# PytorchConnectomics/pytorch_connectomics

Measured on AMD Instinct MI355X. Metric: voxels/s (train + sliding-window infer), MedNeXt-S 112^3 bf16, higher is better.
Workload: dtype bf16; 1 GPU; Lucchi++ sliding-window inference (configs[1]): MedNeXt-S k3, 165x1024x768 volume, roi 112^3, overlap 0.5, bump blending, sw_batch_size 8, random-init weights; step = one whole-volume EagerSlidingWindowEngine call (TTA off); value = window-voxels/s; sw_batch_size=8, window_pipeline_streams=3

## Files before the change

### include/pytc_hip.h

```cpp
#ifndef PYTC_HIP_H
#define PYTC_HIP_H

#include <stdint.h>

#ifdef __cplusplus
extern "C" {
#endif

#define PYTC_ABI_VERSION 5

#define PYTC_OK 0
#define PYTC_ERR_INVALID 1
#define PYTC_ERR_HIP 2
#define PYTC_ERR_UNSUPPORTED 3

#define PYTC_F32 0
#define PYTC_BF16 1

#define PYTC_VIEW_FLIP_Z 1
#define PYTC_VIEW_FLIP_Y 2
#define PYTC_VIEW_FLIP_X 4
#define PYTC_VIEW_SWAP_YX 8
#define PYTC_VIEW_SWAP_ZY 16
#define PYTC_VIEW_SWAP_ZX 32
// ... 80 lines not shown
#define PYTC_NORM_MINMAX 2
#define PYTC_NORM_DIVIDE 3
int64_t pytc_window_normalize_ws_elems(int B, int64_t n);
int pytc_window_normalize(float* x, int B, int64_t n, int mode, int binarize, float threshold, float divide, const float* clip,
                          double* workspace, void* stream);


int pytc_dwconv3d_stat_slots(int N, int D, int H, int W, int C, int K, int stride, int dtype,
                             int transposed);

int pytc_dwconv3d_kernel_variant(int N, int D, int H, int W, int C, int K, int stride, int dtype, int transposed);

int pytc_dwconv3d_fwd(const void* x, void* y, const float* w, const float* bias, float* stats,
                      int N, int D, int H, int W, int C, int K, int stride, int dtype,
                      void* stream);

int pytc_dwconv3d_fwd_wide(const void* x, void* y, const float* w, const float* bias, float* stats, int N, int D, int H,
                           int W, int C, int K, int stride, int dtype, void* stream);

int pytc_dwconv3d_res_supported(int D, int H, int W, int C, int K, int stride, int dtype);

int pytc_dwmix_supported(int D, int H, int W, int C, int C_hid, int C_out, int dtype);
int pytc_dwmix_fwd(const void* x, const float* taps, const float* dw_bias, const void* w2n, const float* b2n, const void* w3_f16,
                   const float* b3, int residual, void* y, const void* head_w, const float* head_b, float* head_y, int n_head, int N,
                   int D, int H, int W, int C, int C_hid, int C_out, int dtype, void* stream);
int pytc_dwconv3d_fwd_res(const void* x, const void* res, void* y, const float* w, const float* bias, int N, int D, int H,
                          int W, int C, int K, int stride, int dtype, void* stream);

int pytc_dwconvT3d_fwd(const void* x, void* y, const float* w, const float* bias, float* stats,
                       int N, int D, int H, int W, int C, int K, int dtype, void* stream);
// ... 325 lines not shown
```

### pytorch_connectomics_amd/_native.py

```python
from __future__ import annotations

import ctypes as C
import os
from pathlib import Path

LIB_PATH = Path(__file__).resolve().parent / "lib" / "libpytc_hip.so"
ABI_VERSION = 5

F32, BF16 = 0, 1
OK = 0

VIEW_FLIP_Z, VIEW_FLIP_Y, VIEW_FLIP_X, VIEW_SWAP_YX, VIEW_SWAP_ZY, VIEW_SWAP_ZX = 1, 2, 4, 8, 16, 32
VIEW_SWAPS = {VIEW_SWAP_YX: (1, 2), VIEW_SWAP_ZY: (0, 1), VIEW_SWAP_ZX: (0, 2)}
PAD_MODES = {"constant": 0, "reflect": 1, "replicate": 2, "circular": 3}
BLEND_PRODUCT, BLEND_MIN = 0, 1
ACT_NONE, ACT_SIGMOID, ACT_TANH, ACT_GELU, ACT_SOFTMAX, ACT_RELU, ACT_LEAKY, ACT_ELU = 0, 1, 2, 3, 4, 5, 6, 7
RES_NONE, RES_ADD, RES_UPSAMPLE, RES_GELU_BWD, RES_NORM_BWD = 0, 1, 2, 3, 4


class PwArgs(C.Structure):
    _fields_ = [
        ("x", C.c_void_p), ("w_packed", C.c_void_p), ("bias", C.c_void_p), ("ab", C.c_void_p),
        ("res", C.c_void_p), ("y", C.c_void_p),
        ("N", C.c_int), ("rows_per_sample", C.c_int64),
# ... 43 lines not shown
    "pytc_gather_windows": (C.c_int, [C.c_void_p, C.c_int, C.c_int, C.c_int, C.c_int, C.POINTER(C.c_int32),
                                      C.c_int, C.c_int, C.c_int, C.c_int, C.c_int, C.c_int, C.c_float,
                                      C.c_void_p, C.c_int, C.c_void_p]),
    "pytc_blend_accumulate": (C.c_int, [C.c_void_p, C.c_int, C.c_int, C.POINTER(C.c_int32), C.c_int, C.c_int,
                                        C.c_int, C.c_int, C.c_int, C.c_void_p, C.c_void_p, C.c_void_p, C.c_int,
                                        C.c_float, C.POINTER(C.c_int32), C.c_void_p, C.c_void_p, C.c_int, C.c_int,
                                        C.c_int, C.c_void_p]),
    "pytc_blend_finalize": (C.c_int, [C.c_void_p, C.c_void_p, C.c_int, C.c_int64, C.c_float, C.c_int, C.c_void_p]),
    "pytc_channel_activation": (C.c_int, [C.c_void_p, C.c_int, C.c_int64, C.c_int, C.c_int, C.c_int, C.c_int,
                                          C.c_float, C.c_void_p]),
    "pytc_ensemble_update": (C.c_int, [C.c_void_p, C.c_void_p, C.c_int64, C.c_int, C.c_int, C.c_void_p]),
    "pytc_dwconv3d_stat_slots": (C.c_int, [C.c_int] * 9),
    "pytc_dwconv3d_kernel_variant": (C.c_int, [C.c_int] * 9),
    "pytc_dwconv3d_fwd": (C.c_int, [C.c_void_p, C.c_void_p, C.c_void_p, C.c_void_p, C.c_void_p] + [C.c_int] * 8
                          + [C.c_void_p]),
    "pytc_dwconv3d_fwd_wide": (C.c_int, [C.c_void_p, C.c_void_p, C.c_void_p, C.c_void_p, C.c_void_p] + [C.c_int] * 8
                               + [C.c_void_p]),
    "pytc_dwconv3d_res_supported": (C.c_int, [C.c_int] * 7),
    "pytc_dwmix_supported": (C.c_int, [C.c_int] * 7),
    "pytc_dwmix_fwd": (C.c_int, [C.c_void_p] * 7 + [C.c_int] + [C.c_void_p] * 4 + [C.c_int] * 9 + [C.c_void_p]),
    "pytc_dwconv3d_fwd_res": (C.c_int, [C.c_void_p, C.c_void_p, C.c_void_p, C.c_void_p, C.c_void_p] + [C.c_int] * 8
                              + [C.c_void_p]),
    "pytc_dwconvT3d_fwd": (C.c_int, [C.c_void_p, C.c_void_p, C.c_void_p, C.c_void_p, C.c_void_p] + [C.c_int] * 7
                           + [C.c_void_p]),
    "pytc_groupnorm_finalize": (C.c_int, [C.c_void_p, C.c_int, C.c_float, C.c_void_p, C.c_void_p, C.c_float,
                                          C.c_void_p, C.c_int, C.c_int, C.c_void_p]),
    "pytc_groupnorm_fold_mlp": (C.c_int, [C.c_void_p, C.c_int, C.c_float, C.c_void_p, C.c_void_p, C.c_float, C.c_void_p,
                                          C.c_void_p, C.c_void_p, C.c_void_p, C.c_void_p, C.c_int, C.c_int, C.c_int, C.c_void_p]),
    "pytc_pw_gemm_supported": (C.c_int, [C.c_int, C.c_int]),
    "pytc_pw_gemm_fwd": (C.c_int, [C.c_void_p, C.c_void_p, C.c_void_p, C.c_void_p, C.c_void_p, C.c_int, C.c_int64, C.c_int, C.c_int,
# ... 248 lines not shown
```

### pytorch_connectomics_amd/csrc/dwconv_kernels.hip

```cpp
#include <type_traits>
#include "pytc_common.h"
#include "dwconv_march.h"

namespace pytc {

struct DwGeom {
  int N, D, H, W, C, K, stride, Do, Ho, Wo;
  int lpv;
  int vs;
  int iters;
  int slots;
  int cell;
  int xblock;
};

template <int VEC>
__device__ __forceinline__ void block_stats_reduce(float (&s1)[VEC], float (&s2)[VEC], int cv, int vslot,
                                                   bool active, const DwGeom& g, float* __restrict__ stats,
                                                   int n, int slot, float* lds) {
  const int C = g.C;
  if (active) {
#pragma unroll
    for (int i = 0; i < VEC; ++i) {
      lds[(vslot * 2 + 0) * C + cv * VEC + i] = s1[i];
// ... 1103 lines not shown
template <typename T>
static int dispatch_vec(int vec, bool transposed, const void* x, void* y, const float* w, const float* bias,
                        float* stats, const DwGeom& g, hipStream_t s) {
  switch (vec) {
    case 8: if constexpr (sizeof(T) == 2) return launch_dw<T, 8>(transposed, x, y, w, bias, stats, g, s); else break;
    case 4: return launch_dw<T, 4>(transposed, x, y, w, bias, stats, g, s);
    case 2: return launch_dw<T, 2>(transposed, x, y, w, bias, stats, g, s);
    case 1: return launch_dw<T, 1>(transposed, x, y, w, bias, stats, g, s);
  }
  set_error("dwconv3d: bad vector width %d", vec);
  return PYTC_ERR_INVALID;
}

static int dw_entry(bool transposed, const void* x, void* y, const float* w, const float* bias, float* stats,
                    int N, int D, int H, int W, int C, int K, int stride, int dtype, void* stream,
                    const void* res = nullptr, bool wide_range = false) {
  PYTC_REQUIRE(x && w, "dwconv3d: null pointer");
  if (res) {
    PYTC_REQUIRE(y && !stats, "dwconv3d_res: needs an output and takes no statistics");
    if (dtype != PYTC_BF16 || !march_ok(D, H, W, C, K, stride, dtype, transposed)) {
      set_error("dwconv3d_res: bf16 only, shape outside the z-march kernel (N=%d D=%d H=%d W=%d C=%d K=%d stride=%d)", N, D, H, W, C, K, stride);
      return PYTC_ERR_UNSUPPORTED;
    }
  }
  PYTC_REQUIRE(N >= 1 && D >= 1 && H >= 1 && W >= 1 && C >= 1, "dwconv3d: bad shape");
  PYTC_REQUIRE(stride == 1 || stride == 2, "dwconv3d: stride must be 1 or 2");
  PYTC_REQUIRE(dtype == PYTC_F32 || dtype == PYTC_BF16, "dwconv3d: bad dtype");
  PYTC_REQUIRE(!(wide_range && stats), "dwconv3d_fwd_wide: the gradient entry computes no statistics");
  DwTTile tt;
  const bool tt_form = transposed && K == 3 && dtype == PYTC_BF16 && (C == 64 || C == 128) && tuning_get("dwconvT_tile", 1) != 0 &&
                       dwconvT_tile_plan(tt, N, D, H, W, C);
// ... 15 lines not shown
    return PYTC_OK;
  }
  if (!transposed && K == 3 && stride == 2 && dtype == PYTC_BF16 && y && tuning_get("dwconv_s2_march", 1) != 0) {
    DwS2 t2;
    if (dwconv_s2_plan(t2, N, D, H, W, C)) {
      dwconv_s2_launch(x, y, w, bias, stats, t2, (hipStream_t)stream);
      PYTC_LAUNCH_CHECK("dwconv3d_k3_s2_march");
      return PYTC_OK;
    }
  }
  if (!res && !wide_range && mfma_small_ok(D, H, W, C, K, stride, dtype, transposed)) {
    DwMarch t;
    make_march(t, N, D, H, W, C, TILE_X);
    t.swizzle = tuning_get("dwconv_xcd_swizzle", 1);
    t.cg_inner = tuning_get("dwconv_cg_inner", 1);
    dwconv_mfma_launch(x, y, w, bias, stats, t, tuning_get("dwconv_mfma_variant", 0) | 1, (hipStream_t)stream);
    PYTC_LAUNCH_CHECK("dwconv3d_k3_mfma");
    return PYTC_OK;
  }
  if (march_ok(D, H, W, C, K, stride, dtype, transposed)) {
    DwMarch t;
    const bool wide_tile = !res && !wide_range && tuning_get("dwconv_march_h16", 1) != 0 && march_tile_x(W, dtype) == 16;
    make_march(t, N, D, H, W, C, wide_tile ? 16 : TILE_X);
    dim3 grid((unsigned)((long)t.slots * (C / MARCH_CG) * N)), block(wide_tile ? 512 : 256);
    t.swizzle = tuning_get("dwconv_xcd_swizzle", 1);
  t.cg_inner = tuning_get("dwconv_cg_inner", 1);
    if (dtype == PYTC_BF16 && !res && !wide_range && tuning_get("dwconv_mfma", 1) != 0) {
      dwconv_mfma_launch(x, y, w, bias, stats, t, tuning_get("dwconv_mfma_variant", 0), (hipStream_t)stream);
      PYTC_LAUNCH_CHECK("dwconv3d_k3_mfma");
      return PYTC_OK;
    }
    const int variant = tuning_get("dwconv_march_variant", 0);
#define PYTC_MARCH(PP, WW) \
  hipLaunchKernelGGL((dwconv3d_k3_march_kernel<bf16_t, 2, PP, true, WW>), grid, block, 0, (hipStream_t)stream, \
                     (const bf16_t*)x, (bf16_t*)y, w, bias, stats, t)
    const int h16 = (res || wide_range) ? 0 : tuning_get("dwconv_march_h16", 1);
    if (res) {
      if (h16)
        hipLaunchKernelGGL((dwconv3d_k3_march_kernel<bf16_t, 2, 3, true, 3, true, true>), grid, block, 0, (hipStream_t)stream,
                           (const bf16_t*)x, (bf16_t*)y, w, bias, stats, t, (const bf16_t*)res);
      else
        hipLaunchKernelGGL((dwconv3d_k3_march_kernel<bf16_t, 2, 3, true, 3, true>), grid, block, 0, (hipStream_t)stream,
                           (const bf16_t*)x, (bf16_t*)y, w, bias, stats, t, (const bf16_t*)res);
// ... 68 lines not shown
  DwGeom g;
  int vec;
  if (!make_geom(g, N, D, H, W, C, K, stride, dtype, transposed, vec)) return -1;
  if (transposed && K == 3 && dtype == PYTC_BF16 && (C == 64 || C == 128) && tuning_get("dwconvT_tile", 1) != 0) return 7;
  if (!transposed && K == 3 && stride == 2 && dtype == PYTC_BF16 && (C == 32 || C == 64) && tuning_get("dwconv_s2_march", 1) != 0) return 8;
  if (transposed) return g.cell ? 4 : 5;
  const size_t taps = (size_t)K * K * K * C * sizeof(float);
  if ((K == 3 || K == 5 || K == 7) && taps <= 64 * 1024 && tuning_get("dwconv_gather", 1) != 0)
    return (vec == 8 && stride == 1 && g.xblock) ? 2 : 1;
  return 0;
}

extern "C" int pytc_dwconv3d_fwd(const void* x, void* y, const float* w, const float* bias, float* stats, int N,
                                 int D, int H, int W, int C, int K, int stride, int dtype, void* stream) {
  return dw_entry(false, x, y, w, bias, stats, N, D, H, W, C, K, stride, dtype, stream);
}

extern "C" int pytc_dwconv3d_fwd_wide(const void* x, void* y, const float* w, const float* bias, float* stats, int N,
                                      int D, int H, int W, int C, int K, int stride, int dtype, void* stream) {
  return dw_entry(false, x, y, w, bias, stats, N, D, H, W, C, K, stride, dtype, stream, nullptr, true);
}

extern "C" int pytc_dwconv3d_res_supported(int D, int H, int W, int C, int K, int stride, int dtype) {
  return (dtype == PYTC_BF16 && march_ok(D, H, W, C, K, stride, dtype, 0)) ? 1 : 0;
}

extern "C" int pytc_dwconv3d_fwd_res(const void* x, const void* res, void* y, const float* w, const float* bias, int N,
                                     int D, int H, int W, int C, int K, int stride, int dtype, void* stream) {
  PYTC_REQUIRE(res, "dwconv3d_res: null residual");
  return dw_entry(false, x, y, w, bias, nullptr, N, D, H, W, C, K, stride, dtype, stream, res);
// ... 55 lines not shown
```

### pytorch_connectomics_amd/csrc/dwconv_march.h

```cpp
#pragma once
#include "pytc_common.h"

namespace pytc {

struct DwMarch {
  int N, D, H, W, C;
  int ty, tx, zc, nzc;
  int tilex;
  int slots;
  int swizzle;
  int cg_inner;
};

void dwconv_mfma_launch(const void* x, void* y, const float* w, const float* bias, float* stats, const DwMarch& g, int variant,
                        hipStream_t s);

struct DwMix {
  const bf16x8_t* w2n;
  const float* b2n;
  const h8_t* w3;
  const float* b3;
  long w2_stride;
  int residual;
  const bf16x8_t* head_w;
  const float* head_b;
  float* head_y;
  int n_head, store_y;
  float* prof;
};
int dwmix_launch(const void* x, void* y, const float* w, const float* bias, const DwMarch& g, const DwMix& mx, int c_hid, int variant,
// ... 12 lines not shown
```

### pytorch_connectomics_amd/csrc/dwconv_mfma_kernels.hip

```cpp
#include <type_traits>

#include "dwconv_march.h"
#include "pw_common.h"

namespace pytc {

typedef short s4_t __attribute__((ext_vector_type(4)));
typedef unsigned int u32x4_t __attribute__((ext_vector_type(4)));
typedef unsigned int u32x2a4_t __attribute__((ext_vector_type(2), aligned(4)));
typedef __bf16 bf2_t __attribute__((ext_vector_type(2)));
typedef float f2_t __attribute__((ext_vector_type(2)));

constexpr int MF_TY = 8, MF_TX = 8, MF_CG = 32;
constexpr int MF_EY = MF_TY + 2, MF_EX = MF_TX + 2;
constexpr int MF_EXP = 16;
constexpr int MF_CS = MF_EY * MF_EXP + 2;
constexpr int MF_IMG = MF_CG * MF_CS;
constexpr int MF_NCHUNK = MF_EY * MF_EX * (MF_CG / 8);
constexpr int MF_CPT = 2;
constexpr int MF_TS = 32;
constexpr int MF_RS = MF_TX * MF_TS + 8;

__device__ __forceinline__ unsigned short mf_bf16_bits(float f) {
  unsigned int u = __float_as_uint(f);
// ... 4 lines not shown

template <int N>
__device__ __forceinline__ void mf_wait_vm() { asm volatile("s_waitcnt vmcnt(%0)" : : "n"(N) : "memory"); }


template <int N>
__device__ __forceinline__ void mf_wait_vm_upto(int n) {
  if constexpr (N > 0) {
    if (n >= N) { mf_wait_vm<N>(); return; }
    mf_wait_vm_upto<N - 1>(n);
  } else {
    mf_wait_vm<0>();
  }
}

template <int PF, bool LO, int PROBE = 0, bool STORE = true, int MIXHC = 0>
__global__ void __launch_bounds__(256, MIXHC ? 3 : 4)
dwconv3d_k3_mfma_kernel(const unsigned short* __restrict__ x, unsigned short* __restrict__ y, const float* __restrict__ w,
                        const float* __restrict__ bias, float* __restrict__ stats, DwMarch g, DwMix mx) {
  static_assert(PF == 2 || PF == 3, "two or three planes in flight");
  static_assert(MIXHC == 0 || (STORE && PF == 3), "the fused block keeps the output tile and three planes in flight");
  constexpr bool MIX = MIXHC > 0;
  __shared__ __attribute__((aligned(16))) bf16x8_t w2s[MIX ? MIXHC * 2 * 64 : 1];
  __shared__ __attribute__((aligned(16))) h8_t w3s[MIX ? 2 * MIXHC * 64 : 1];
  __shared__ __attribute__((aligned(16))) float mbias[MIX ? 32 * MIXHC + 32 : 4];
  __shared__ __attribute__((aligned(16))) unsigned short image[2][MF_IMG];
  __shared__ __attribute__((aligned(16))) unsigned short otile[STORE ? 2 : 1][STORE ? MF_TY * MF_RS : 8];
  __shared__ float wl[27 * MF_CG];
  __shared__ float red[4][2][16];

  const int tid = threadIdx.x, wave = tid >> 6, lane = tid & 63;
  int b = g.swizzle ? xcd_swizzle(blockIdx.x, gridDim.x) : blockIdx.x;
  const int ncg = g.C / MF_CG;
  const int cg = g.cg_inner ? b % ncg : (b / g.slots) % ncg;
  const int slot_id = g.cg_inner ? (b / ncg) % g.slots : b % g.slots;
  const int n = b / (ncg * g.slots);
  b = slot_id;
  const int fx = b % g.tx; b /= g.tx;
  const int fy = b % g.ty;
  const int zchunk = b / g.ty;
  const int y0 = fy * MF_TY, x0 = fx * MF_TX;
  const int zs = zchunk * g.zc;
  const int ze = min(zs + g.zc, g.D);
  const int C = g.C;
// ... 277 lines not shown
      tk[7] = __builtin_amdgcn_s_memtime() - tstart;
      float* o = stats + (((long)n * g.slots + slot_id) * 2) * C + cg * MF_CG + wave * 8;
#pragma unroll
      for (int k = 0; k < 8; ++k) o[k] = (float)tk[k];
    }
    return;
  }
  if (!MIX && stats) {
    s1 += __shfl_xor(s1, 1, 64); s2 += __shfl_xor(s2, 1, 64);
    s1 += __shfl_xor(s1, 2, 64); s2 += __shfl_xor(s2, 2, 64);
    if (j == 0) { red[wave][0][cl] = s1; red[wave][1][cl] = s2; }
    __syncthreads();
    if (tid < 2 * MF_CG) {
      const int which = tid / MF_CG, chn = tid % MF_CG;
      const float a = red[chn >> 4][which][chn & 15] + red[(chn >> 4) + 2][which][chn & 15];
      stats[(((long)n * g.slots + slot_id) * 2 + which) * C + cg * MF_CG + chn] = a;
    }
  }
}

void dwconv_mfma_launch(const void* x, void* y, const float* w, const float* bias, float* stats, const DwMarch& g, int variant,
                        hipStream_t s) {
  dim3 grid((unsigned)((long)g.slots * (g.C / MF_CG) * g.N)), block(256);
  const unsigned short* xp = (const unsigned short*)x;
  unsigned short* yp = (unsigned short*)y;
  const DwMix none{};
#define PYTC_MF(PFV, LOV, NM) hipLaunchKernelGGL((dwconv3d_k3_mfma_kernel<PFV, LOV, NM>), grid, block, 0, s, xp, yp, w, bias, stats, g, none)
#define PYTC_MF_STATS(PFV, LOV) hipLaunchKernelGGL((dwconv3d_k3_mfma_kernel<PFV, LOV, 0, false>), grid, block, 0, s, xp, yp, w, bias, stats, g, none)
  const int probe = tuning_get("dwconv_mfma_probe", 0);
  if (!y) {
    if (variant & 1) { if (variant & 2) PYTC_MF_STATS(2, true); else PYTC_MF_STATS(3, true); }
    else { if (variant & 2) PYTC_MF_STATS(2, false); else PYTC_MF_STATS(3, false); }
  }
  else if (probe == 1) PYTC_MF(3, false, 1);
  else if (probe == 3) PYTC_MF(3, false, 3);
  else if (probe == 4) PYTC_MF(3, false, 4);
  else if (variant & 1) { if (variant & 2) PYTC_MF(2, true, 0); else PYTC_MF(3, true, 0); }
  else { if (variant & 2) PYTC_MF(2, false, 0); else PYTC_MF(3, false, 0); }
#undef PYTC_MF
#undef PYTC_MF_STATS
}

int dwmix_launch(const void* x, void* y, const float* w, const float* bias, const DwMarch& g, const DwMix& mx, int c_hid, int variant,
                 hipStream_t s) {
  dim3 grid((unsigned)((long)g.slots * g.N)), block(256);
  const unsigned short* xp = (const unsigned short*)x;
  unsigned short* yp = (unsigned short*)y;
#define PYTC_DM(LOV, HCV, PRB) hipLaunchKernelGGL((dwconv3d_k3_mfma_kernel<3, LOV, PRB, true, HCV>), grid, block, 0, s, xp, yp, w, bias, (float*)nullptr, g, mx)
  const bool lo = variant & 1;
  if (mx.prof) {
    if (c_hid != 64 || lo) return -1;
    PYTC_DM(false, 2, 4);
    return 0;
  }
  switch (c_hid) {
    case 64: if (lo) PYTC_DM(true, 2, 0); else PYTC_DM(false, 2, 0); break;
    case 96: if (lo) PYTC_DM(true, 3, 0); else PYTC_DM(false, 3, 0); break;
    case 128: if (lo) PYTC_DM(true, 4, 0); else PYTC_DM(false, 4, 0); break;
    default: return -1;
  }
#undef PYTC_DM
  return 0;
}
// ... 3 lines not shown
```

### pytorch_connectomics_amd/hip_ops.py

```python
from __future__ import annotations

import ctypes as C
from typing import Optional, Sequence

import torch

from . import _native as nat

_DT = {torch.float32: nat.F32, torch.bfloat16: nat.BF16}


def dtype_code(dt: torch.dtype) -> int:
    try:
        return _DT[dt]
    except KeyError:
        raise TypeError(f"pytorch_connectomics_amd kernels support float32/bfloat16, got {dt}") from None


def require_device(device, what: str = "this inference path") -> None:
    if torch.device(device).type != "cuda":
        raise RuntimeError(f"{what} (pytorch_connectomics_amd) needs a CUDA(HIP) device: there is no CPU path")


def _dev(t: torch.Tensor, name: str) -> torch.Tensor:
# ... 262 lines not shown
        if slots < 0:
            raise RuntimeError(f"dwconv3d: unsupported channel count {Cc}")
        st = torch.empty((N, slots, 2, Cc), dtype=torch.float32, device=x.device)
    tag = f"C{Cc}_k{K}" + ("_s2" if stride == 2 and not transposed else "")
    if transposed:
        _run(f"dwconvT3d_fwd[{tag}]" if store else f"dwconvT3d_stats[{tag}]", _nbytes(x, y), nat.lib().pytc_dwconvT3d_fwd, _p(x), _p(y), _p(w_taps), _p(bias),
             _p(st), N, D, H, W, Cc, K, dt, _stream())
    else:
        sym = None
        if PROFILER.enabled:
            sym = _DW_VARIANTS.get(nat.lib().pytc_dwconv3d_kernel_variant(N, D, H, W, Cc, K, stride, dt, 0))
        fn = nat.lib().pytc_dwconv3d_fwd_wide if wide_range else nat.lib().pytc_dwconv3d_fwd
        _run(f"dwconv3d_fwd[{tag}]" if store else f"dwconv3d_stats[{tag}]", _nbytes(x, y), fn, _p(x), _p(y), _p(w_taps), _p(bias),
             _p(st), N, D, H, W, Cc, K, stride, dt, _stream(), symbol=sym)
    return y, st


_DW_VARIANTS = {0: "dwconv3d_direct_kernel", 1: "dwconv3d_k3_gather_kernel", 2: "dwconv3d_xblock_kernel",
                3: "dwconv3d_k3_march_kernel", 4: "dwconvT3d_k3_cell_kernel", 5: "dwconvT3d_kernel",
                6: "dwconv3d_k3_mfma_kernel", 7: "dwconvT3d_k3_tile_kernel", 8: "dwconv3d_k3_s2_march_kernel"}


def dwconv3d_res_supported(x: torch.Tensor, K: int, stride: int = 1) -> bool:
    N, D, H, W, Cc = x.shape
    return bool(nat.lib().pytc_dwconv3d_res_supported(D, H, W, Cc, K, stride, dtype_code(x.dtype)))


def dwconv3d_res(x: torch.Tensor, w_taps: torch.Tensor, res: torch.Tensor, *, K: int = 3) -> torch.Tensor:
    _dev(x, "x"); _dev(res, "res"); _dev(w_taps, "w_taps")
    if res.shape != x.shape or res.dtype != x.dtype:
# ... 1778 lines not shown
```

### pytorch_connectomics_amd/models/architectures/mednext.py

```python
from __future__ import annotations

import os
from typing import Dict, List, Optional, Sequence, Union

import torch
import torch.nn as nn

from ... import _native as nat
from ... import hip_ops as ops

SMALL_ROWS_TWO_GEMMS = int(os.environ.get("PYTC_MIXER_TWO_GEMM_ROWS", "0"))

L0_SUBBATCH = int(os.environ.get("PYTC_L0_SUBBATCH", "0"))


def _conv_nd(dim: str):
    if dim == "3d":
        return nn.Conv3d, nn.ConvTranspose3d
    if dim == "2d":
        return nn.Conv2d, nn.ConvTranspose2d
    raise ValueError(f"dim must be '2d' or '3d', got {dim!r}")


class _ChannelLayerNorm(nn.Module):
# ... 99 lines not shown

class HipBlockOps:

    def __init__(self):
        self.cache = _WeightCache()
        self.fused = True
        self.fuse_up = os.environ.get("PYTC_FUSE_UP", "0") == "1"
        self.fuse_up_cin = (64, 128)
        self.fold_norm = os.environ.get("PYTC_FOLD_NORM", "1") != "0"
        self.deep_gemm_rows = int(os.environ.get("PYTC_DEEP_GEMM_ROWS", "8192"))
        self.deep_gemm_cin = int(os.environ.get("PYTC_DEEP_GEMM_CIN", "0"))
        self.lds_mixer_rows = int(os.environ.get("PYTC_LDS_MIXER_ROWS", "131072"))
        self.chunk_mixer_rows = int(os.environ.get("PYTC_CHUNK_MIXER_ROWS", "16384"))
        self.chunk_mixer_hid = int(os.environ.get("PYTC_CHUNK_MIXER_HID", "512"))
        self.fuse_block = int(os.environ.get("PYTC_FUSE_BLOCK", "0"))

    def _taps(self, conv: nn.Module):
        w = conv.weight
        def make():
            c = w.shape[0]
            k = w.shape[-1]
            w3 = embed_stencil_2d(w.detach().float()) if w.dim() == 4 else w.detach().float()
            return w3.reshape(c, k ** 3).t().contiguous(), k
        return self.cache.get(("taps", id(conv)), [w], make)

    def _pw(self, conv: nn.Module, dt: torch.dtype, transposed: bool = False):
        w = conv.weight
        def make():
            w2 = w.detach().float().reshape(w.shape[0], w.shape[1]).contiguous()
            return ops.pw_pack_weight(w2, dt, transposed=transposed)
# ... 92 lines not shown
        b1 = self._vec(m.conv1, "bias", m.conv1.bias)
        kind = m.kind
        c_hid = m.conv2.weight.shape[0]
        c_out = m.conv3.weight.shape[0]
        if (kind == "up" and self.fused and self.fuse_up and C in self.fuse_up_cin and dt == torch.bfloat16 and K == 3 and not m.grn and not is_ln
                and m.dim == "3d"
                and skip is not None and m.conv2.bias is not None and m.conv3.bias is not None
                and ops.pw_mlp_up_supported(C, c_hid, c_out)):
            return self._up_block_fused(m, x, skip, taps, b1, c_hid, c_out)
        if (kind == "block" and self.fused and self.fuse_block and self.fold_norm and dt == torch.bfloat16 and K == 3 and not m.grn and not is_ln
                and m.dim == "3d" and m.conv2.bias is not None and m.conv3.bias is not None and ops.MLP_F16_PROJECT
                and ops.dwmix_supported(x, c_hid, c_out) and ops.groupnorm_fold_mlp_supported(C, c_hid)
                and proj is None
                and (head is None or (head.weight.shape[1] <= 16 and ops.pw_mlp_head_supported(C, c_hid, c_out)))):
            return self._block_dwmix(m, x, taps, b1, c_hid, c_out, head, out)
        if kind == "up":
            t, st = ops.dwconv3d(x, taps, b1, K=K, transposed=True, stats=not is_ln)
            count = float((2 * D - 1) * (2 * H - 1) * (2 * W - 1))
        else:
            t, st = ops.dwconv3d(x, taps, b1, K=K, stride=2 if kind == "down" else 1, stats=not is_ln)
            count = float(t.shape[1] * t.shape[2] * t.shape[3])
        gamma, beta = self._vec(m.norm, "weight", m.norm.weight), self._vec(m.norm, "bias", m.norm.bias)
        if is_ln:
            t = ops.layernorm_rows(t, gamma, beta, m.norm.eps)
            ab = None
        else:
            ab = None
        _, Do, Ho, Wo, _ = t.shape
        rows = Do * Ho * Wo
        small = (self.fused and dt == torch.bfloat16 and not m.grn and not is_ln and N * rows < SMALL_ROWS_TWO_GEMMS
                 and ops.pw_conv_paired_supported(c_in=C, c_out=c_hid, in_dtype=dt, out_dtype=dt)
                 and ops.pw_conv_paired_supported(c_in=c_hid, c_out=c_out, in_dtype=dt, out_dtype=dt))
        if (not small and self.fused and dt == torch.bfloat16 and not m.grn and not is_ln and m.conv2.bias is not None
                and m.conv3.bias is not None and head is None and ops.MLP_F16_PROJECT
                and (rows <= self.deep_gemm_rows or (self.deep_gemm_cin and C >= self.deep_gemm_cin))
                and ops.pw_gemm_supported(C, c_hid) and ops.pw_gemm_supported(c_hid, c_out)):
            ab = ops.groupnorm_finalize(st, count, gamma, beta, m.norm.eps)
            return self._block_deep_gemm(m, x, t, ab, skip, (N, D, H, W, C), (Do, Ho, Wo), c_hid, c_out, out)
        if (not small and self.fused and dt == torch.bfloat16 and not m.grn and not is_ln and m.conv2.bias is not None
                and m.conv3.bias is not None and ops.pw_mlp_supported(C, c_hid, c_out)):
            ab, w2x, b2x = self._fold(m, st, count, C, c_hid)
            if (head is not None and kind == "block" and head.weight.shape[1] <= 16
                    and ops.pw_mlp_head_supported(C, c_hid, c_out)):
                _, logits = ops.pw_mlp_head(t, ab, w2x, b2x,
                                            self._pw_paired(m.conv3, project=True), self._vec(m.conv3, "bias", m.conv3.bias),
                                            self._head_w(head), self._vec(head, "bias", head.bias), N=N,
                                            rows_per_sample=rows, c_in=C, c_hid=c_hid, c_out=c_out,
                                            res=x if m.do_res else None, store_y=False)
                return None, logits.view(N, Do, Ho, Wo, -1)
            if (proj is not None and head is None and out is None and kind == "block" and ab is None and ops.MLP_F16_PROJECT
                    and tuple(proj.weight.shape[:2]) == (32, c_out) and ops.pw_mlp_proj_supported(C, c_hid, c_out, 32)):
                _, z = ops.pw_mlp_proj(t, w2x, b2x, self._pw_paired(m.conv3, project=True), self._vec(m.conv3, "bias", m.conv3.bias),
                                       self._pw_paired(proj), self._vec(proj, "bias", proj.bias), N=N, rows_per_sample=rows, c_in=C,
                                       c_hid=c_hid, c_out=c_out, res=x if m.do_res else None, store_y=False)
                return None, z.view(N, Do, Ho, Wo, 32)
            return self._block_fused(m, x, t, ab, skip, (N, D, H, W, C), (Do, Ho, Wo), c_hid, c_out, out, w2x, b2x)
# ... 448 lines not shown
```

Measured before the change: 1.814 billion voxels/s.

## Fuse GroupNorm finalize and weight fold into dwconv kernel via last-block tail

Adds a tail to the MFMA depthwise conv kernel. Each block publishes its partial statistics and bumps a per-sample arrival counter, and the last block to arrive computes the GroupNorm scale/shift, or folds the norm into the conv2 weights and bias. This removes the separate finalize/fold kernel launches and their round trip between kernels in each MedNeXt block. In exchange, one block per sample does serial reduction work at the end, the kernel uses more shared memory and registers, and correctness now depends on counters being reset and not shared across concurrent streams.

```diff
diff --git a/include/pytc_hip.h b/include/pytc_hip.h
--- a/include/pytc_hip.h
+++ b/include/pytc_hip.h
@@ -118,6 +118,12 @@
 int pytc_dwconv3d_fwd(const void* x, void* y, const float* w, const float* bias, float* stats,
                       int N, int D, int H, int W, int C, int K, int stride, int dtype,
                       void* stream);
+
+int pytc_dwconv3d_norm_tail_supported(int N, int D, int H, int W, int C, int K, int stride, int dtype, int C_hid);
+int pytc_dwconv3d_fwd_norm(const void* x, void* y, const float* w, const float* bias, float* stats, unsigned int* counter,
+                           float count, const float* gamma, const float* beta, float eps, const float* w2, const float* b2,
+                           void* w2n, float* b2n, float* ab, int C_hid, int N, int D, int H, int W, int C, int K, int stride,
+                           int dtype, void* stream);
 
 int pytc_dwconv3d_fwd_wide(const void* x, void* y, const float* w, const float* bias, float* stats, int N, int D, int H,
                            int W, int C, int K, int stride, int dtype, void* stream);
diff --git a/pytorch_connectomics_amd/_native.py b/pytorch_connectomics_amd/_native.py
--- a/pytorch_connectomics_amd/_native.py
+++ b/pytorch_connectomics_amd/_native.py
@@ -81,6 +81,9 @@
     "pytc_dwconv3d_kernel_variant": (C.c_int, [C.c_int] * 9),
     "pytc_dwconv3d_fwd": (C.c_int, [C.c_void_p, C.c_void_p, C.c_void_p, C.c_void_p, C.c_void_p] + [C.c_int] * 8
                           + [C.c_void_p]),
+    "pytc_dwconv3d_norm_tail_supported": (C.c_int, [C.c_int] * 9),
+    "pytc_dwconv3d_fwd_norm": (C.c_int, [C.c_void_p] * 6 + [C.c_float, C.c_void_p, C.c_void_p, C.c_float] + [C.c_void_p] * 5
+                               + [C.c_int] * 9 + [C.c_void_p]),
     "pytc_dwconv3d_fwd_wide": (C.c_int, [C.c_void_p, C.c_void_p, C.c_void_p, C.c_void_p, C.c_void_p] + [C.c_int] * 8
                                + [C.c_void_p]),
     "pytc_dwconv3d_res_supported": (C.c_int, [C.c_int] * 7),
diff --git a/pytorch_connectomics_amd/csrc/dwconv_kernels.hip b/pytorch_connectomics_amd/csrc/dwconv_kernels.hip
--- a/pytorch_connectomics_amd/csrc/dwconv_kernels.hip
+++ b/pytorch_connectomics_amd/csrc/dwconv_kernels.hip
@@ -1,6 +1,7 @@
 #include <type_traits>
 #include "pytc_common.h"
 #include "dwconv_march.h"
+#include "norm_tail.h"
 
 namespace pytc {
 
@@ -1141,7 +1142,7 @@
 
 static int dw_entry(bool transposed, const void* x, void* y, const float* w, const float* bias, float* stats,
                     int N, int D, int H, int W, int C, int K, int stride, int dtype, void* stream,
-                    const void* res = nullptr, bool wide_range = false) {
+                    const void* res = nullptr, bool wide_range = false, const NormTail* tail = nullptr) {
   PYTC_REQUIRE(x && w, "dwconv3d: null pointer");
   if (res) {
     PYTC_REQUIRE(y && !stats, "dwconv3d_res: needs an output and takes no statistics");
@@ -1187,7 +1188,7 @@
     make_march(t, N, D, H, W, C, TILE_X);
     t.swizzle = tuning_get("dwconv_xcd_swizzle", 1);
     t.cg_inner = tuning_get("dwconv_cg_inner", 1);
-    dwconv_mfma_launch(x, y, w, bias, stats, t, tuning_get("dwconv_mfma_variant", 0) | 1, (hipStream_t)stream);
+    dwconv_mfma_launch(x, y, w, bias, stats, t, tuning_get("dwconv_mfma_variant", 0) | 1, (hipStream_t)stream, tail);
     PYTC_LAUNCH_CHECK("dwconv3d_k3_mfma");
     return PYTC_OK;
   }
@@ -1199,7 +1200,7 @@
     t.swizzle = tuning_get("dwconv_xcd_swizzle", 1);
   t.cg_inner = tuning_get("dwconv_cg_inner", 1);
     if (dtype == PYTC_BF16 && !res && !wide_range && tuning_get("dwconv_mfma", 1) != 0) {
-      dwconv_mfma_launch(x, y, w, bias, stats, t, tuning_get("dwconv_mfma_variant", 0), (hipStream_t)stream);
+      dwconv_mfma_launch(x, y, w, bias, stats, t, tuning_get("dwconv_mfma_variant", 0), (hipStream_t)stream, tail);
       PYTC_LAUNCH_CHECK("dwconv3d_k3_mfma");
       return PYTC_OK;
     }
@@ -1298,6 +1299,29 @@
 extern "C" int pytc_dwconv3d_fwd(const void* x, void* y, const float* w, const float* bias, float* stats, int N,
                                  int D, int H, int W, int C, int K, int stride, int dtype, void* stream) {
   return dw_entry(false, x, y, w, bias, stats, N, D, H, W, C, K, stride, dtype, stream);
+}
+
+extern "C" int pytc_dwconv3d_norm_tail_supported(int N, int D, int H, int W, int C, int K, int stride, int dtype, int C_hid) {
+  if (N < 1 || dtype != PYTC_BF16 || tuning_get("dwconv_mfma", 1) == 0 || tuning_get("dwconv_mfma_probe", 0) != 0) return 0;
+  if (!march_ok(D, H, W, C, K, stride, dtype, 0) && !mfma_small_ok(D, H, W, C, K, stride, dtype, 0)) return 0;
+  if (C_hid > 0) return ((C == 32 || C == 64 || C == 128) && C_hid % 32 == 0 && C_hid <= 512) ? 1 : 0;
+  DwMarch t;
+  make_march(t, N, D, H, W, C, TILE_X);
+  return (C_hid == 0 && C % 16 == 0 && t.slots <= 128) ? 1 : 0;
+}
+
+extern "C" int pytc_dwconv3d_fwd_norm(const void* x, void* y, const float* w, const float* bias, float* stats, unsigned int* counter,
+                                      float count, const float* gamma, const float* beta, float eps, const float* w2, const float* b2,
+                                      void* w2n, float* b2n, float* ab, int C_hid, int N, int D, int H, int W, int C, int K,
+                                      int stride, int dtype, void* stream) {
+  PYTC_REQUIRE(y && stats && counter && count > 0, "dwconv3d_fwd_norm: output, statistics and arrival counters are required");
+  PYTC_REQUIRE(pytc_dwconv3d_norm_tail_supported(N, D, H, W, C, K, stride, dtype, w2 ? C_hid : 0),
+               "dwconv3d_fwd_norm: shape outside the norm tail (N=%d D=%d H=%d W=%d C=%d K=%d stride=%d C_hid=%d)", N, D, H, W, C, K, stride, C_hid);
+  PYTC_REQUIRE(w2 ? (w2n && b2n && C_hid > 0) : ab != nullptr, "dwconv3d_fwd_norm: fold needs w2n / b2n, finalize needs ab");
+  NormTail tl{};
+  tl.counter = counter; tl.gamma = gamma; tl.beta = beta; tl.eps = eps; tl.count = count;
+  tl.w2 = w2; tl.b2 = b2; tl.w2n = (bf16_t*)w2n; tl.b2n = b2n; tl.ab = ab; tl.C_hid = C_hid;
+  return dw_entry(false, x, y, w, bias, stats, N, D, H, W, C, K, stride, dtype, stream, nullptr, false, &tl);
 }
 
 extern "C" int pytc_dwconv3d_fwd_wide(const void* x, void* y, const float* w, const float* bias, float* stats, int N,
diff --git a/pytorch_connectomics_amd/csrc/dwconv_march.h b/pytorch_connectomics_amd/csrc/dwconv_march.h
--- a/pytorch_connectomics_amd/csrc/dwconv_march.h
+++ b/pytorch_connectomics_amd/csrc/dwconv_march.h
@@ -12,8 +12,9 @@
   int cg_inner;
 };
 
+struct NormTail;
 void dwconv_mfma_launch(const void* x, void* y, const float* w, const float* bias, float* stats, const DwMarch& g, int variant,
-                        hipStream_t s);
+                        hipStream_t s, const NormTail* tail = nullptr);
 
 struct DwMix {
   const bf16x8_t* w2n;
diff --git a/pytorch_connectomics_amd/csrc/dwconv_mfma_kernels.hip b/pytorch_connectomics_amd/csrc/dwconv_mfma_kernels.hip
--- a/pytorch_connectomics_amd/csrc/dwconv_mfma_kernels.hip
+++ b/pytorch_connectomics_amd/csrc/dwconv_mfma_kernels.hip
@@ -2,6 +2,7 @@
 
 #include "dwconv_march.h"
 #include "pw_common.h"
+#include "norm_tail.h"
 
 namespace pytc {
 
@@ -42,11 +43,12 @@
   }
 }
 
-template <int PF, bool LO, int PROBE = 0, bool STORE = true, int MIXHC = 0>
+template <int PF, bool LO, int PROBE = 0, bool STORE = true, int MIXHC = 0, bool TAIL = false>
 __global__ void __launch_bounds__(256, MIXHC ? 3 : 4)
 dwconv3d_k3_mfma_kernel(const unsigned short* __restrict__ x, unsigned short* __restrict__ y, const float* __restrict__ w,
-                        const float* __restrict__ bias, float* __restrict__ stats, DwMarch g, DwMix mx) {
+                        const float* __restrict__ bias, float* __restrict__ stats, DwMarch g, DwMix mx, NormTail tl) {
   static_assert(PF == 2 || PF == 3, "two or three planes in flight");
+  static_assert(!TAIL || (STORE && MIXHC == 0 && PROBE == 0), "the norm tail rides on the plain storing kernel");
   static_assert(MIXHC == 0 || (STORE && PF == 3), "the fused block keeps the output tile and three planes in flight");
   constexpr bool MIX = MIXHC > 0;
   __shared__ __attribute__((aligned(16))) bf16x8_t w2s[MIX ? MIXHC * 2 * 64 : 1];
@@ -56,6 +58,7 @@
   __shared__ __attribute__((aligned(16))) unsigned short otile[STORE ? 2 : 1][STORE ? MF_TY * MF_RS : 8];
   __shared__ float wl[27 * MF_CG];
   __shared__ float red[4][2][16];
+  __shared__ unsigned int tail_flag[1];
 
   const int tid = threadIdx.x, wave = tid >> 6, lane = tid & 63;
   int b = g.swizzle ? xcd_swizzle(blockIdx.x, gridDim.x) : blockIdx.x;
@@ -363,21 +366,39 @@
     if (tid < 2 * MF_CG) {
       const int which = tid / MF_CG, chn = tid % MF_CG;
       const float a = red[chn >> 4][which][chn & 15] + red[(chn >> 4) + 2][which][chn & 15];
-      stats[(((long)n * g.slots + slot_id) * 2 + which) * C + cg * MF_CG + chn] = a;
+      float* dst = &stats[(((long)n * g.slots + slot_id) * 2 + which) * C + cg * MF_CG + chn];
+      if constexpr (TAIL) norm_tail_store(dst, a);
+      else *dst = a;
+    }
+    if constexpr (TAIL) {
+      asm volatile("s_waitcnt vmcnt(0)" ::: "memory");
+      if (!norm_tail_arrive(tl, n, (unsigned)(g.slots * ncg), tail_flag)) return;
+      static_assert(sizeof(image) >= 4096 * 4 && sizeof(otile) >= 2048 * 4 && sizeof(wl) >= 512 * 4, "norm tail scratch");
+      if (tl.w2)
+        norm_tail_fold<256>(stats, g.slots, n, C, tl, reinterpret_cast<float*>(&image[0][0]), reinterpret_cast<float*>(&otile[0][0]), wl);
+      else
+        norm_tail_finalize<256>(stats, g.slots, n, C, tl);
+      norm_tail_reset(tl, n);
     }
   }
 }
 
 void dwconv_mfma_launch(const void* x, void* y, const float* w, const float* bias, float* stats, const DwMarch& g, int variant,
-                        hipStream_t s) {
+                        hipStream_t s, const NormTail* tail) {
   dim3 grid((unsigned)((long)g.slots * (g.C / MF_CG) * g.N)), block(256);
   const unsigned short* xp = (const unsigned short*)x;
   unsigned short* yp = (unsigned short*)y;
   const DwMix none{};
-#define PYTC_MF(PFV, LOV, NM) hipLaunchKernelGGL((dwconv3d_k3_mfma_kernel<PFV, LOV, NM>), grid, block, 0, s, xp, yp, w, bias, stats, g, none)
-#define PYTC_MF_STATS(PFV, LOV) hipLaunchKernelGGL((dwconv3d_k3_mfma_kernel<PFV, LOV, 0, false>), grid, block, 0, s, xp, yp, w, bias, stats, g, none)
+  const NormTail nt = tail ? *tail : NormTail{};
+#define PYTC_MF(PFV, LOV, NM) hipLaunchKernelGGL((dwconv3d_k3_mfma_kernel<PFV, LOV, NM>), grid, block, 0, s, xp, yp, w, bias, stats, g, none, nt)
+#define PYTC_MF_STATS(PFV, LOV) hipLaunchKernelGGL((dwconv3d_k3_mfma_kernel<PFV, LOV, 0, false>), grid, block, 0, s, xp, yp, w, bias, stats, g, none, nt)
+#define PYTC_MF_TAIL(PFV, LOV) hipLaunchKernelGGL((dwconv3d_k3_mfma_kernel<PFV, LOV, 0, true, 0, true>), grid, block, 0, s, xp, yp, w, bias, stats, g, none, nt)
   const int probe = tuning_get("dwconv_mfma_probe", 0);
-  if (!y) {
+  if (tail) {
+    if (variant & 1) { if (variant & 2) PYTC_MF_TAIL(2, true); else PYTC_MF_TAIL(3, true); }
+    else { if (variant & 2) PYTC_MF_TAIL(2, false); else PYTC_MF_TAIL(3, false); }
+  }
+  else if (!y) {
     if (variant & 1) { if (variant & 2) PYTC_MF_STATS(2, true); else PYTC_MF_STATS(3, true); }
     else { if (variant & 2) PYTC_MF_STATS(2, false); else PYTC_MF_STATS(3, false); }
   }
@@ -388,6 +409,7 @@
   else { if (variant & 2) PYTC_MF(2, false, 0); else PYTC_MF(3, false, 0); }
 #undef PYTC_MF
 #undef PYTC_MF_STATS
+#undef PYTC_MF_TAIL
 }
 
 int dwmix_launch(const void* x, void* y, const float* w, const float* bias, const DwMarch& g, const DwMix& mx, int c_hid, int variant,
@@ -395,7 +417,7 @@
   dim3 grid((unsigned)((long)g.slots * g.N)), block(256);
   const unsigned short* xp = (const unsigned short*)x;
   unsigned short* yp = (unsigned short*)y;
-#define PYTC_DM(LOV, HCV, PRB) hipLaunchKernelGGL((dwconv3d_k3_mfma_kernel<3, LOV, PRB, true, HCV>), grid, block, 0, s, xp, yp, w, bias, (float*)nullptr, g, mx)
+#define PYTC_DM(LOV, HCV, PRB) hipLaunchKernelGGL((dwconv3d_k3_mfma_kernel<3, LOV, PRB, true, HCV>), grid, block, 0, s, xp, yp, w, bias, (float*)nullptr, g, mx, NormTail{})
   const bool lo = variant & 1;
   if (mx.prof) {
     if (c_hid != 64 || lo) return -1;
diff --git a/pytorch_connectomics_amd/csrc/norm_tail.h b/pytorch_connectomics_amd/csrc/norm_tail.h
--- /dev/null
+++ b/pytorch_connectomics_amd/csrc/norm_tail.h
@@ -0,0 +1,168 @@
+#pragma once
+#include "pw_common.h"
+
+namespace pytc {
+
+struct NormTail {
+  unsigned int* counter;
+  const float* gamma;
+  const float* beta;
+  float eps, count;
+  const float* w2;
+  const float* b2;
+  bf16_t* w2n;
+  float* b2n;
+  float* ab;
+  int C_hid;
+};
+
+__device__ __forceinline__ void norm_tail_store(float* p, float v) {
+  __hip_atomic_store(p, v, __ATOMIC_RELAXED, __HIP_MEMORY_SCOPE_AGENT);
+}
+
+__device__ __forceinline__ bool norm_tail_arrive(const NormTail& tl, int n, unsigned int arrivals, unsigned int* flag) {
+  if (threadIdx.x == 0) *flag = __hip_atomic_fetch_add(tl.counter + n, 1u, __ATOMIC_RELAXED, __HIP_MEMORY_SCOPE_AGENT);
+  __syncthreads();
+  if (*flag != arrivals - 1) return false;
+  __builtin_amdgcn_fence(__ATOMIC_ACQUIRE, "agent");
+  asm volatile("s_waitcnt vmcnt(0)" ::: "memory");
+  __syncthreads();
+  return true;
+}
+
+__device__ __forceinline__ void norm_tail_reset(const NormTail& tl, int n) {
+  if (threadIdx.x == 0) __hip_atomic_store(tl.counter + n, 0u, __ATOMIC_RELAXED, __HIP_MEMORY_SCOPE_AGENT);
+}
+
+template <int NT>
+__device__ __forceinline__ void norm_tail_finalize(const float* stats, int slots, int n, int C, const NormTail& tl) {
+  const float* base = stats + (long)n * slots * 2 * C;
+  for (int c = threadIdx.x; c < C; c += NT) {
+    float t1 = 0.f, t2 = 0.f;
+    for (int wave = 0; wave < 16; ++wave) {
+      float p1[4], p2[4];
+#pragma unroll
+      for (int q = 0; q < 4; ++q) {
+        float a1 = 0.f, a2 = 0.f;
+        for (int s = wave * 4 + q; s < slots; s += 64) {
+          a1 += base[((long)s * 2 + 0) * C + c];
+          a2 += base[((long)s * 2 + 1) * C + c];
+        }
+        p1[q] = a1;
+        p2[q] = a2;
+      }
+      float a1 = p1[0], a2 = p2[0];
+      a1 += p1[1]; a2 += p2[1];
+      const float o1 = p1[2] + p1[3], o2 = p2[2] + p2[3];
+      a1 += o1; a2 += o2;
+      t1 += a1; t2 += a2;
+    }
+    const float count = tl.count, eps = tl.eps;
+    float mean = t1 / count;
+    float var = fmaxf(t2 / count - mean * mean, 0.f);
+    float rstd = rsqrtf(var + eps);
+    rstd = rstd * (1.5f - 0.5f * (var + eps) * rstd * rstd);
+    float a = (tl.gamma ? tl.gamma[c] : 1.f) * rstd;
+    float b = (tl.beta ? tl.beta[c] : 0.f) - mean * a;
+    tl.ab[((long)n * 2 + 0) * C + c] = a;
+    tl.ab[((long)n * 2 + 1) * C + c] = b;
+  }
+}
+
+template <int NT>
+__device__ __forceinline__ void norm_tail_fold(const float* stats, int slots, int n, int C, const NormTail& tl, float* red, float* part,
+                                               float* vec) {
+  static_assert(1024 % NT == 0, "the stand-alone kernel's 1024 threads in whole passes");
+  float* sa = vec; float* sb = vec + 128; float* smean = vec + 256; float* sbeta = vec + 384;
+  const int Q = C / 2, SL = 1024 / Q;
+  const int C_hid = tl.C_hid;
+  const float* w2 = tl.w2;
+  for (int vt = threadIdx.x; vt < 1024; vt += NT) {
+    const int col = vt % Q, sl = vt / Q;
+    const float* base = stats + (long)n * slots * 2 * C + col * 4;
+    f32x4_t a = {0.f, 0.f, 0.f, 0.f};
+    constexpr int INFL = 8;
+    for (int s0 = sl; s0 < slots; s0 += SL * INFL) {
+      f32x4_t v[INFL];
+#pragma unroll
+      for (int i = 0; i < INFL; ++i) {
+        const int s = s0 + i * SL;
+        v[i] = s < slots ? *reinterpret_cast<const f32x4_t*>(base + (long)s * 2 * C) : f32x4_t{0.f, 0.f, 0.f, 0.f};
+      }
+#pragma unroll
+      for (int i = 0; i < INFL; ++i)
+        if (s0 + i * SL < slots) a += v[i];
+    }
+    *reinterpret_cast<f32x4_t*>(&red[vt * 4]) = a;
+  }
+  __syncthreads();
+  const int groups = 1024 / (2 * C) < 8 ? 1024 / (2 * C) : 8;
+  for (int vt = threadIdx.x; vt < 1024; vt += NT) {
+    const int e = vt % (2 * C), pg = vt / (2 * C);
+    if (pg < groups) {
+      float t = 0.f;
+      for (int s = pg; s < SL; s += groups) t += red[s * 2 * C + e];
+      part[pg * 256 + e] = t;
+    }
+  }
+  __syncthreads();
+  for (int vt = threadIdx.x; vt < C; vt += NT) {
+    const float count = tl.count, eps = tl.eps;
+    float t1 = 0.f, t2 = 0.f;
+    for (int g = 0; g < groups; ++g) { t1 += part[g * 256 + vt]; t2 += part[g * 256 + C + vt]; }
+    const float mean = t1 / count;
+    const float var = fmaxf(t2 / count - mean * mean, 0.f);
+    float rstd = rsqrtf(var + eps);
+    rstd = rstd * (1.5f - 0.5f * (var + eps) * rstd * rstd);
+    const float av = (tl.gamma ? tl.gamma[vt] : 1.f) * rstd;
+    const float bv = (tl.beta ? tl.beta[vt] : 0.f) - mean * av;
+    sa[vt] = av;
+    sb[vt] = bv;
+    smean[vt] = mean;
+    sbeta[vt] = tl.beta ? tl.beta[vt] : 0.f;
+    if (tl.ab) {
+      tl.ab[((long)n * 2 + 0) * C + vt] = av;
+      tl.ab[((long)n * 2 + 1) * C + vt] = bv;
+    }
+  }
+  __syncthreads();
+  const int KG = C / 32;
+  const long total = (long)C_hid * C;
+  bf16_t* img = tl.w2n + (long)n * total;
+  for (long e8 = threadIdx.x; e8 < total / 8; e8 += NT) {
+    long t = e8;
+    const int lane = (int)(t % 64);
+    t /= 64;
+    const int kg = (int)(t % KG);
+    const int T = (int)(t / KG);
+    const int o = paired_row(T, lane & 15);
+    const int k = kg * 32 + (lane >> 4) * 8;
+    float v[8];
+    VecIO<float, 4>::load(w2 + (long)o * C + k, reinterpret_cast<float(&)[4]>(v[0]));
+    VecIO<float, 4>::load(w2 + (long)o * C + k + 4, reinterpret_cast<float(&)[4]>(v[4]));
+#pragma unroll
+    for (int j = 0; j < 8; ++j) v[j] *= sa[k + j];
+    *reinterpret_cast<bf16x8_t*>(img + e8 * 8) = Mma<bf16_t>::from_floats(v);
+  }
+  for (int o = threadIdx.x; o < C_hid; o += NT) {
+    float acc = tl.b2 ? tl.b2[o] : 0.f;
+    const float* wr = w2 + (long)o * C;
+    for (int k = 0; k < C; k += 8) {
+      const f32x4_t w0 = *reinterpret_cast<const f32x4_t*>(wr + k), w1 = *reinterpret_cast<const f32x4_t*>(wr + k + 4);
+      float v[8], wn[8];
+#pragma unroll
+      for (int j = 0; j < 4; ++j) { v[j] = w0[j] * sa[k + j]; v[4 + j] = w1[j] * sa[k + 4 + j]; }
+      const bf16x8_t rounded = Mma<bf16_t>::from_floats(v);
+      VecIO<bf16_t, 8>::load(reinterpret_cast<const bf16_t*>(&rounded), wn);
+#pragma unroll
+      for (int j = 0; j < 8; ++j) {
+        const float wj = j < 4 ? w0[j] : w1[j - 4];
+        acc = fmaf(wj, sbeta[k + j], acc);
+        acc = fmaf(-wn[j], smean[k + j], acc);
+      }
+    }
+    tl.b2n[(long)n * C_hid + o] = acc;
+  }
+}
+
+}
diff --git a/pytorch_connectomics_amd/hip_ops.py b/pytorch_connectomics_amd/hip_ops.py
--- a/pytorch_connectomics_amd/hip_ops.py
+++ b/pytorch_connectomics_amd/hip_ops.py
@@ -300,6 +300,51 @@
         _run(f"dwconv3d_fwd[{tag}]" if store else f"dwconv3d_stats[{tag}]", _nbytes(x, y), fn, _p(x), _p(y), _p(w_taps), _p(bias),
              _p(st), N, D, H, W, Cc, K, stride, dt, _stream(), symbol=sym)
     return y, st
+
+
+NORM_TAIL_MAX_N = 1024
+_TAIL_COUNTERS = {}
+
+
+def _tail_counter(device: torch.device) -> torch.Tensor:
+    key = (device.index, _stream().value)
+    c = _TAIL_COUNTERS.get(key)
+    if c is None:
+        c = _TAIL_COUNTERS[key] = torch.zeros(NORM_TAIL_MAX_N, dtype=torch.int32, device=device)
+    return c
+
+
+def dwconv3d_norm_supported(x: torch.Tensor, K: int, c_hid: int = 0) -> bool:
+    N, D, H, W, Cc = x.shape
+    if not x.is_cuda or x.dtype != torch.bfloat16 or N > NORM_TAIL_MAX_N:
+        return False
+    return bool(nat.lib().pytc_dwconv3d_norm_tail_supported(N, D, H, W, Cc, K, 1, nat.BF16, int(c_hid)))
+
+
+def dwconv3d_norm(x: torch.Tensor, w_taps: torch.Tensor, bias: Optional[torch.Tensor], *, K: int, count: float,
+                  gamma: Optional[torch.Tensor], beta: Optional[torch.Tensor], eps: float, w2: Optional[torch.Tensor] = None,
+                  b2: Optional[torch.Tensor] = None, want_ab: bool = False):
+    _dev(x, "x"); _dev(w_taps, "w_taps")
+    N, D, H, W, Cc = x.shape
+    c_hid = 0 if w2 is None else int(w2.shape[0])
+    if not dwconv3d_norm_supported(x, K, c_hid):
+        raise ValueError(f"dwconv3d_norm: unsupported problem {tuple(x.shape)} {x.dtype} K={K} c_hid={c_hid}")
+    if w2 is not None and (w2.dtype != torch.float32 or tuple(w2.shape) != (c_hid, Cc) or not w2.is_contiguous()):
+        raise ValueError(f"dwconv3d_norm: w2 must be contiguous fp32 (C_hid, {Cc}), got {tuple(w2.shape)} {w2.dtype}")
+    y = torch.empty_like(x)
+    slots = nat.lib().pytc_dwconv3d_stat_slots(N, D, H, W, Cc, K, 1, nat.BF16, 0)
+    st = torch.empty((N, slots, 2, Cc), dtype=torch.float32, device=x.device)
+    ab = torch.empty((N, 2, Cc), dtype=torch.float32, device=x.device) if (w2 is None or want_ab) else None
+    w2n = b2n = None
+    if w2 is not None:
+        w2n = torch.empty((N, c_hid * Cc), dtype=torch.bfloat16, device=x.device)
+        b2n = torch.empty((N, c_hid), dtype=torch.float32, device=x.device)
+    _run(f"dwconv3d_fwd[C{Cc}_k{K}]", _nbytes(x, y), nat.lib().pytc_dwconv3d_fwd_norm, _p(x), _p(y), _p(w_taps), _p(bias), _p(st),
+         _p(_tail_counter(x.device)), float(count), _p(gamma), _p(beta), float(eps), _p(w2), _p(b2), _p(w2n), _p(b2n), _p(ab), c_hid,
+         N, D, H, W, Cc, K, 1, nat.BF16, _stream(), symbol="dwconv3d_k3_mfma_kernel")
+    if w2 is None:
+        return y, st, ab
+    return (y, st, w2n, b2n, ab) if want_ab else (y, st, w2n, b2n)
 
 
 _DW_VARIANTS = {0: "dwconv3d_direct_kernel", 1: "dwconv3d_k3_gather_kernel", 2: "dwconv3d_xblock_kernel",
diff --git a/pytorch_connectomics_amd/models/architectures/mednext.py b/pytorch_connectomics_amd/models/architectures/mednext.py
--- a/pytorch_connectomics_amd/models/architectures/mednext.py
+++ b/pytorch_connectomics_amd/models/architectures/mednext.py
@@ -137,6 +137,7 @@
         self.chunk_mixer_rows = int(os.environ.get("PYTC_CHUNK_MIXER_ROWS", "16384"))
         self.chunk_mixer_hid = int(os.environ.get("PYTC_CHUNK_MIXER_HID", "512"))
         self.fuse_block = int(os.environ.get("PYTC_FUSE_BLOCK", "0"))
+        self.norm_tail = os.environ.get("PYTC_NORM_TAIL", "1") != "0"
 
     def _taps(self, conv: nn.Module):
         w = conv.weight
@@ -259,6 +260,10 @@
                 and proj is None
                 and (head is None or (head.weight.shape[1] <= 16 and ops.pw_mlp_head_supported(C, c_hid, c_out)))):
             return self._block_dwmix(m, x, taps, b1, c_hid, c_out, head, out)
+        if (kind == "block" and self.norm_tail and dt == torch.bfloat16 and not is_ln and m.dim == "3d"):
+            y = self._block_any_tail(m, x, head, out, proj)
+            if y is not None:
+                return y
         if kind == "up":
             t, st = ops.dwconv3d(x, taps, b1, K=K, transposed=True, stats=not is_ln)
             count = float((2 * D - 1) * (2 * H - 1) * (2 * W - 1))
@@ -266,6 +271,39 @@
             t, st = ops.dwconv3d(x, taps, b1, K=K, stride=2 if kind == "down" else 1, stats=not is_ln)
             count = float(t.shape[1] * t.shape[2] * t.shape[3])
         gamma, beta = self._vec(m.norm, "weight", m.norm.weight), self._vec(m.norm, "bias", m.norm.bias)
+        return self._block_mix(m, x, t, st, count, gamma, beta, skip, head, out, proj, is_ln)
+
+    def _block_any_tail(self, m: MedNeXtBlock, x: torch.Tensor, head, out, proj):
+        N, D, H, W, C = x.shape
+        taps, K = self._taps(m.conv1)
+        c_hid, c_out = m.conv2.weight.shape[0], m.conv3.weight.shape[0]
+        rows = D * H * W
+        if (not self.fused or K != 3 or m.grn or m.conv2.bias is None or m.conv3.bias is None or N * rows < SMALL_ROWS_TWO_GEMMS):
+            return None
+        gamma, beta = self._vec(m.norm, "weight", m.norm.weight), self._vec(m.norm, "bias", m.norm.bias)
+        b1 = self._vec(m.conv1, "bias", m.conv1.bias)
+        deep = (head is None and ops.MLP_F16_PROJECT and (rows <= self.deep_gemm_rows or (self.deep_gemm_cin and C >= self.deep_gemm_cin))
+                and ops.pw_gemm_supported(C, c_hid) and ops.pw_gemm_supported(c_hid, c_out))
+        if deep:
+            if not ops.dwconv3d_norm_supported(x, K, 0):
+                return None
+            t, st, ab = ops.dwconv3d_norm(x, taps, b1, K=K, count=float(rows), gamma=gamma, beta=beta, eps=m.norm.eps)
+            pre = (ab, None, None)
+        elif (ops.pw_mlp_supported(C, c_hid, c_out) and self.fold_norm and ops.groupnorm_fold_mlp_supported(C, c_hid)
+              and ops.dwconv3d_norm_supported(x, K, c_hid)):
+            t, st, w2n, b2n = ops.dwconv3d_norm(x, taps, b1, K=K, count=float(rows), gamma=gamma, beta=beta, eps=m.norm.eps,
+                                                w2=self._w2_matrix(m.conv2), b2=self._vec(m.conv2, "bias", m.conv2.bias))
+            pre = (None, w2n, b2n)
+        else:
+            return None
+        return self._block_mix(m, x, t, st, float(rows), gamma, beta, None, head, out, proj, False, pre=pre)
+
+    def _block_mix(self, m, x, t, st, count, gamma, beta, skip, head, out, proj, is_ln, pre=None):
+        dt = x.dtype
+        N, D, H, W, C = x.shape
+        kind = m.kind
+        c_hid = m.conv2.weight.shape[0]
+        c_out = m.conv3.weight.shape[0]
         if is_ln:
             t = ops.layernorm_rows(t, gamma, beta, m.norm.eps)
             ab = None
@@ -280,11 +318,11 @@
                 and m.conv3.bias is not None and head is None and ops.MLP_F16_PROJECT
                 and (rows <= self.deep_gemm_rows or (self.deep_gemm_cin and C >= self.deep_gemm_cin))
                 and ops.pw_gemm_supported(C, c_hid) and ops.pw_gemm_supported(c_hid, c_out)):
-            ab = ops.groupnorm_finalize(st, count, gamma, beta, m.norm.eps)
+            ab = pre[0] if pre is not None else ops.groupnorm_finalize(st, count, gamma, beta, m.norm.eps)
             return self._block_deep_gemm(m, x, t, ab, skip, (N, D, H, W, C), (Do, Ho, Wo), c_hid, c_out, out)
         if (not small and self.fused and dt == torch.bfloat16 and not m.grn and not is_ln and m.conv2.bias is not None
                 and m.conv3.bias is not None and ops.pw_mlp_supported(C, c_hid, c_out)):
-            ab, w2x, b2x = self._fold(m, st, count, C, c_hid)
+            ab, w2x, b2x = pre if pre is not None else self._fold(m, st, count, C, c_hid)
             if (head is not None and kind == "block" and head.weight.shape[1] <= 16
                     and ops.pw_mlp_head_supported(C, c_hid, c_out)):
                 _, logits = ops.pw_mlp_head(t, ab, w2x, b2x,
```

Measured after the change: 1.808 billion voxels/s. About the same (-0.3%).
